# mdnunez/bayesflow_nddms

Hardware: AMD Instinct MI355X
Metric: simulated DDM trials/sec at n_trials=300 dt=0.001 (basic_ddm_dc, max_steps=4000) (higher is better)
Workload: dtype f32

## Files before the change

### bayesflow_nddms_amd/_lib.py

```python
import ctypes
import os

from .build import SO_PATH

NDDM_OK, NDDM_ERR_NULL, NDDM_ERR_SHAPE, NDDM_ERR_PARAM, NDDM_ERR_HIP, NDDM_ERR_NO_DEVICE = range(6)
GAUSS_EXACT, GAUSS_FAST, BRIDGE, GAUSS_PACKED, STATE_F64 = 0, 1, 2, 4, 8
QUANTILE_CONDITIONAL = 1
HMC_SIGMA_FIXED = 1
ABI_VERSION = 4

_lib = None


class NddmLibraryError(ImportError):
    pass


def _declare(L):
    c = ctypes
    fp, vp = c.c_void_p, c.c_void_p
    L.nddm_abi_version.restype = c.c_int
    L.nddm_last_error.restype = c.c_char_p
    L.nddm_device_count.argtypes = [c.POINTER(c.c_int)]
    L.nddm_set_device.argtypes = [c.c_int]
    L.nddm_summary_k.restype = c.c_int
    L.nddm_model_nparams.argtypes = [c.c_int]
    L.nddm_set_tuning.argtypes = [c.c_int] * 6
    L.nddm_set_debug_trace.argtypes = [c.c_void_p, c.c_int, c.c_int]
    L.nddm_set_ordering.argtypes = [c.c_int]
    L.nddm_debug_set_slot_limit.argtypes = [c.c_int]
    L.nddm_debug_last_launch.argtypes = [c.POINTER(c.c_int32)]
    common = [c.c_int64, c.c_int32, c.c_float, c.c_int32, c.c_uint64, c.c_uint64, c.c_uint32]
    for name in ("nddm_basic_ddm_dc_simulate", "nddm_single_trial_simulate", "nddm_single_trial_alt_simulate"):
        getattr(L, name).argtypes = [fp] + common + [fp, fp, vp]
    L.nddm_alpha_not_scaled_simulate.argtypes = [fp] + common + [c.c_float, c.c_int32, fp, fp, fp, vp]
    L.nddm_explicit_boundary_simulate.argtypes = [fp, fp] + common + [fp, fp, vp]
    L.nddm_simulratcliff.argtypes = [fp, c.c_int64, c.c_int32, c.c_uint64, c.c_uint64, c.c_uint32, c.c_float, c.c_int32, fp, fp, fp, vp]
    L.nddm_wiener_log_likelihood.argtypes = [c.c_int32, fp, c.c_int64, c.c_int64, fp, c.c_int32, c.c_uint32, fp, fp, vp]
    L.nddm_wiener_cdf.argtypes = [c.c_int32, fp, c.c_int64, c.c_int64, fp, c.c_int32, c.c_uint32, fp, fp, vp]
    L.nddm_wiener_log_likelihood_grad.argtypes = [c.c_int32, fp, c.c_int64, c.c_int64, fp, c.c_int32, c.c_uint32, fp, fp, vp]
    L.nddm_wiener_marginal_log_likelihood.argtypes = [c.c_int32, fp, c.c_int64, c.c_int64, fp, c.c_int32, c.c_float, c.c_uint32, fp, fp, vp]
    L.nddm_wiener_marginal_log_likelihood_grad.argtypes = [c.c_int32, fp, c.c_int64, c.c_int64, fp, c.c_int32, c.c_float, c.c_uint32, fp, fp, vp]
    L.nddm_wiener_hmc.argtypes = [c.c_int32, fp, c.c_int64, c.c_int32, c.c_int64, c.c_int64, fp, fp, c.c_int32, c.c_int32, c.c_int32, c.c_int32,
                                  c.c_uint32, c.c_uint64, c.c_uint64, c.c_uint64, c.c_uint32, fp, fp, fp, fp, fp, vp]
    L.nddm_wiener_hmc_joint.argtypes = [c.c_int32, fp, c.c_int64, c.c_int32, c.c_int64, c.c_int64, fp, fp, fp, fp, fp, c.c_int32, c.c_int32, c.c_int32,
                                        c.c_int32, c.c_uint32, c.c_uint64, c.c_uint64, c.c_uint64, c.c_uint32, fp, fp, fp, fp, fp, fp, fp, vp]
    L.nddm_wiener_quantile.argtypes = [c.c_int32, fp, c.c_int64, c.c_int64, fp, c.c_int32, c.c_uint32, fp, vp]
    L.nddm_simulate.argtypes = [c.c_int32, fp, fp] + common + [c.c_float, c.c_int32, fp, fp, fp, vp]
    L.nddm_simulate_indirect.argtypes = [c.c_int32, fp, fp] + common[:-1] + [fp, c.c_uint32, c.c_float, c.c_int32, fp, fp, fp, vp]
    L.nddm_simulate_codes.argtypes = [c.c_int32, fp] + common[:-1] + [fp, c.c_uint32, fp, fp, fp, vp]
    L.nddm_decode_codes.argtypes = [c.c_int32, fp, fp, c.c_int64, c.c_int32, c.c_float, fp, vp]
    L.nddm_draw_prior.argtypes = [c.c_int32, c.c_int64, c.c_uint64, c.c_uint64, c.c_float, fp, vp]
    L.nddm_draw_prior_indirect.argtypes = [c.c_int32, c.c_int64, c.c_uint64, c.c_uint64, fp, c.c_float, fp, vp]
    L.nddm_graph_arena_create.argtypes = [c.POINTER(c.c_uint64)]
    L.nddm_graph_arena_bind.argtypes = [c.c_uint64, c.POINTER(c.c_uint64)]
    L.nddm_graph_arena_info.argtypes = [c.c_uint64, c.POINTER(c.c_uint64), c.POINTER(c.c_int32)]
    L.nddm_graph_arena_release.argtypes = [c.c_uint64]
    L.nddm_source_hash.restype = c.c_char_p
    L.nddm_build_info.restype = c.c_char_p
    L.nddm_debug_normals.argtypes = [fp, c.c_int64, c.c_uint32, c.c_uint32, c.c_uint32, fp, vp]
    for name in EXPORTS:
        if name not in ("nddm_last_error", "nddm_source_hash", "nddm_build_info"):
            getattr(L, name).restype = c.c_int


EXPORTS = [
    "nddm_abi_version", "nddm_last_error", "nddm_device_count", "nddm_set_device", "nddm_summary_k",
    "nddm_model_nparams", "nddm_basic_ddm_dc_simulate", "nddm_single_trial_simulate",
    "nddm_single_trial_alt_simulate", "nddm_alpha_not_scaled_simulate", "nddm_explicit_boundary_simulate",
    "nddm_simulate", "nddm_draw_prior", "nddm_debug_normals", "nddm_set_tuning", "nddm_set_debug_trace", "nddm_set_ordering",
    "nddm_release_graph_memory", "nddm_debug_set_slot_limit", "nddm_debug_last_launch",
    "nddm_simulate_indirect", "nddm_draw_prior_indirect", "nddm_source_hash", "nddm_simulate_codes", "nddm_decode_codes",
    "nddm_graph_arena_create", "nddm_graph_arena_bind", "nddm_graph_arena_info", "nddm_graph_arena_release", "nddm_build_info",
    "nddm_simulratcliff", "nddm_wiener_log_likelihood", "nddm_wiener_cdf", "nddm_wiener_quantile",
    "nddm_wiener_log_likelihood_grad", "nddm_wiener_marginal_log_likelihood", "nddm_wiener_marginal_log_likelihood_grad",
    "nddm_wiener_hmc", "nddm_wiener_hmc_joint",
]


def lib():
    global _lib
    if _lib is None:
        from .build import build_hip, embedded_hash, is_stale, source_hash
        override = bool(os.environ.get("NDDM_HIP_LIB"))
        if is_stale():
            try:
                build_hip()
            except Exception as e:
                why = "is missing" if not os.path.exists(SO_PATH) else \
                    f"was built from other sources (library {embedded_hash()}, tree {source_hash()})"
                raise NddmLibraryError(
                    f"{SO_PATH} {why} and could not be rebuilt ({e!r}): build it with "
                    "`python -c 'import __graft_entry__ as g; g.build()'` (hipcc --offload-arch=gfx950).  "
                    "There is no CPU fallback.") from e
        if not os.path.exists(SO_PATH):
            raise NddmLibraryError(f"{SO_PATH} does not exist (NDDM_HIP_LIB points to a missing file?).  There is no CPU fallback.")
        import torch
        try:
            L = ctypes.CDLL(SO_PATH)
        except OSError as e:
            raise NddmLibraryError(f"cannot load {SO_PATH}: {e}") from e
        missing = [name for name in EXPORTS if not hasattr(L, name)]
        if missing:
            raise NddmLibraryError(f"{SO_PATH} does not export {missing}: it is older than this binding -- rebuild it "
                                   "(`python -c 'import __graft_entry__ as g; g.build()'`)")
        _declare(L)
        if L.nddm_abi_version() != ABI_VERSION:
            raise NddmLibraryError(f"ABI mismatch: library {L.nddm_abi_version()} != binding {ABI_VERSION} "
                                   "(the random stream differs between ABI versions): rebuild the library")
        if not override and L.nddm_source_hash().decode() != source_hash():
            raise NddmLibraryError(f"{SO_PATH} reports source hash {L.nddm_source_hash().decode()} but the tree hashes to "
                                   f"{source_hash()}: rebuild the library")
        _lib = L
    return _lib


def check(rc):
    if rc == NDDM_OK:
        return
    msg = lib().nddm_last_error().decode() or f"nddm status {rc}"
    if rc in (NDDM_ERR_NULL, NDDM_ERR_SHAPE, NDDM_ERR_PARAM):
        raise ValueError(msg)
    raise RuntimeError(msg)
```

### bayesflow_nddms_amd/build.py

```python
import hashlib
import os
import re
import shutil
import subprocess

_HERE = os.path.dirname(os.path.abspath(__file__))
SO_PATH = os.environ.get("NDDM_HIP_LIB") or os.path.join(_HERE, "libnddm_hip.so")
SOURCES = [os.path.join(_HERE, "csrc", "nddm_kernels.hip")]
HEADERS = [os.path.join(_HERE, "csrc", "nddm_rng.h"), os.path.join(_HERE, "csrc", "nddm_sim.h"),
           os.path.join(_HERE, "csrc", "nddm_prepass.h"), os.path.join(_HERE, "csrc", "nddm_ratcliff.h"),
           os.path.join(_HERE, "csrc", "nddm_wiener.h"), os.path.join(_HERE, "csrc", "nddm_wiener_cdf.h"),
           os.path.join(_HERE, "csrc", "nddm_wiener_quantile.h"), os.path.join(_HERE, "csrc", "nddm_wiener_grad.h"),
           os.path.join(_HERE, "csrc", "nddm_wiener_marginal.h"), os.path.join(_HERE, "csrc", "nddm_wiener_marginal_grad.h"),
           os.path.join(_HERE, "csrc", "nddm_wiener_hmc.h"),
           os.path.join(_HERE, "csrc", "nddm_wiener_hmc_joint.h"),
           os.path.join(os.path.dirname(_HERE), "include", "nddm.h")]
HIPCC_FLAGS = ["-O3", "-ffp-contract=off", "--offload-arch=gfx950", "-fPIC", "-shared", "-std=c++17"]


def _hipcc():
    exe = shutil.which("hipcc") or "/opt/rocm/bin/hipcc"
    if not os.path.exists(exe):
        raise RuntimeError("hipcc not found: the HIP extension cannot be built")
    return exe


def source_hash():
    h = hashlib.sha256()
    for p in SOURCES + HEADERS:
        h.update(os.path.basename(p).encode() + b"\0")
        with open(p, "rb") as f:
            h.update(f.read())
        h.update(b"\0")
    h.update(" ".join(HIPCC_FLAGS).encode())
    return h.hexdigest()


def embedded_hash(path=None):
    path = path or SO_PATH
    try:
        with open(path, "rb") as f:
            m = re.search(rb"NDDM_SRC_HASH=([0-9a-f]{64})", f.read())
# ... 89 lines not shown
```

### bayesflow_nddms_amd/csrc/nddm_kernels.hip

```cpp
#include <hip/hip_runtime.h>
#include <math.h>
#include <stdint.h>
#include <stdio.h>
#include <stdlib.h>
#include <string.h>

#include <mutex>
#include <thread>

#include "../../include/nddm.h"
#include "nddm_prepass.h"
#include "nddm_ratcliff.h"
#include "nddm_rng.h"
#include "nddm_sim.h"
#include "nddm_wiener.h"
#include "nddm_wiener_cdf.h"
#include "nddm_wiener_grad.h"
#include "nddm_wiener_hmc.h"
#include "nddm_wiener_hmc_joint.h"
#include "nddm_wiener_marginal.h"
#include "nddm_wiener_marginal_grad.h"
#include "nddm_wiener_quantile.h"

namespace nddm {

static thread_local char g_err[512] = "";

static int fail(int code, const char *fmt, const char *detail = "")
{
    snprintf(g_err, sizeof g_err, fmt, detail);
    return code;
}

static int round_up_pow2(int v) { int p = 1; while (p < v) p <<= 1; return p; }

static int check_stream(hipStream_t st)
{
    int sdev = -1, cur = -1;
    const hipError_t e = hipStreamGetDevice(st, &sdev);
    if (e != hipSuccess) {
        (void)hipGetLastError();
        return fail(NDDM_ERR_HIP, "`stream` is not a live stream of this process's HIP runtime (destroyed, or created by another copy "
                                  "of the runtime): %s", hipGetErrorString(e));
    }
    if (hipGetDevice(&cur) == hipSuccess && st != nullptr && st != hipStreamPerThread && sdev != cur)
        return fail(NDDM_ERR_PARAM, "`stream` belongs to another device than the current one (nddm_set_device / hipSetDevice)%s");
    return NDDM_OK;
}

struct Tuning { int sets_per_chunk, ring, refill_thresh, variant, grid_waves, tile_trials, no_order; };
struct LastLaunch { int grid_waves, vkeys, ring, tile_trials, tiles_per_set, sets_per_chunk, refill_thresh, lds_bytes; };
static thread_local LastLaunch g_last = {0, 0, 0, 0, 0, 0, 0, 0};
static std::mutex g_mu;
static Tuning g_tuning = {0, 0, 0, 0, 0, 0, 0};
static unsigned long long *g_dbg = nullptr;
static int g_dbg_waves = 0, g_dbg_chunks = 0;

constexpr int MAX_DEVICES = 64;
struct DeviceInfo { int cus = 0; double clock_hz = 0.0; };
static DeviceInfo g_dev[MAX_DEVICES];

static bool device_info(int dev, DeviceInfo *out)
{
    std::lock_guard<std::mutex> lock(g_mu);
    if (g_dev[dev].cus == 0) {
        hipDeviceProp_t prop;
        if (hipGetDeviceProperties(&prop, dev) != hipSuccess) return false;
        g_dev[dev].cus = prop.multiProcessorCount > 0 ? prop.multiProcessorCount : 1;
        g_dev[dev].clock_hz = prop.clockRate > 0 ? (double)prop.clockRate * 1e3 : 2.4e9;
    }
    *out = g_dev[dev];
    return true;
}

constexpr size_t SLOT_QUEUE_BYTES = 256, SLOT_SCRATCH = 1u << 20;
constexpr int MAX_SLOTS = 256;
struct LaunchSlot {
    char *base = nullptr;
    hipEvent_t done = nullptr;
    hipStream_t stream = nullptr;
    bool busy = false;
    bool fresh = true;
};
static LaunchSlot *g_slots[MAX_DEVICES][MAX_SLOTS];
static int g_nslots[MAX_DEVICES];
static int g_slot_limit = MAX_SLOTS;

static hipError_t malloc_relaxed(void **p, size_t bytes)
{
// ... 221 lines not shown
    }
    if (B < 0 || n_trials <= 0 || max_steps < 0) return fail(NDDM_ERR_SHAPE, "B < 0, n_trials <= 0 or max_steps < 0%s");
    if (max_steps >= (1 << 30)) return fail(NDDM_ERR_SHAPE, "max_steps must be < 2^30%s");
    if (set_offset >= (1ull << 60) || set_offset + (uint64_t)B > (1ull << 60))
        return fail(NDDM_ERR_SHAPE, "set_offset + B must be <= 2^60 (the random stream is keyed by 60 bits of the set index)%s");
    if (!(dt > 0.0f) || !isfinite(dt)) return fail(NDDM_ERR_PARAM, "dt must be finite and > 0%s");
    if (flags > 15u) return fail(NDDM_ERR_PARAM, "unknown flags%s");
    const bool bridge = (flags & NDDM_BRIDGE) != 0;
    const bool packed = (flags & NDDM_GAUSS_PACKED) != 0;
    const bool f64 = (flags & NDDM_STATE_F64) != 0;
    if (f64 && ((model != NDDM_BASIC_DDM_DC && model != NDDM_SINGLE_TRIAL) || bridge || packed || out_codes))
        return fail(NDDM_ERR_PARAM, "NDDM_STATE_F64 exists for NDDM_BASIC_DDM_DC and NDDM_SINGLE_TRIAL, without NDDM_BRIDGE, NDDM_GAUSS_PACKED "
                                    "or the 2-byte wire format%s");
    if (packed && (bridge || max_steps >= 16384))
        return fail(NDDM_ERR_PARAM, "NDDM_GAUSS_PACKED needs max_steps < 2^14 and cannot be combined with NDDM_BRIDGE%s");
    if (bridge && model != NDDM_ALPHA_NOT_SCALED)
        return fail(NDDM_ERR_PARAM, "NDDM_BRIDGE is only available for NDDM_ALPHA_NOT_SCALED%s");
    if (bridge && max_steps >= (1 << 22)) return fail(NDDM_ERR_SHAPE, "max_steps must be < 2^22 with NDDM_BRIDGE%s");
    if (B == 0) return NDDM_OK;
    if (!params) return fail(NDDM_ERR_NULL, "params is NULL%s");
    if (model == NDDM_EXPLICIT_BOUNDARY && !bounds) return fail(NDDM_ERR_NULL, "bounds is NULL%s");
    if (!out_trials && !out_summary && !out_ext && !out_codes) return fail(NDDM_ERR_NULL, "no output buffer given%s");
    if (out_codes && ((model != NDDM_BASIC_DDM_DC && model != NDDM_ALPHA_NOT_SCALED) || bridge || packed || max_steps >= 16384))
        return fail(NDDM_ERR_PARAM, "the 2-byte wire format exists for NDDM_BASIC_DDM_DC and NDDM_ALPHA_NOT_SCALED without NDDM_BRIDGE "
                                    "or NDDM_GAUSS_PACKED, max_steps < 2^14%s");
    if (B * (((long long)n_trials + 511) / 512) >= (1ll << 31))
        return fail(NDDM_ERR_SHAPE, "B * ceil(n_trials / 512) must be < 2^31 per launch%s");

    if (const int rc = check_stream(reinterpret_cast<hipStream_t>(stream))) return rc;

    Tuning tun;
    unsigned long long *dbg;
    int dbg_waves, dbg_chunks;
    { std::lock_guard<std::mutex> lock(g_mu); tun = g_tuning; dbg = g_dbg; dbg_waves = g_dbg_waves; dbg_chunks = g_dbg_chunks; }
    int dev = 0;
    {
        const hipError_t e = hipGetDevice(&dev);
        if (e != hipSuccess || dev < 0 || dev >= MAX_DEVICES) return fail(NDDM_ERR_HIP, "hipGetDevice: %s", hipGetErrorString(e));
    }
    DeviceInfo di;
    if (!device_info(dev, &di)) return fail(NDDM_ERR_HIP, "hipGetDeviceProperties failed%s");
    const int simds = 4 * di.cus;
    static const int sizing_per_simd = [] { const char *e = getenv("NDDM_SIZING_WAVES_PER_SIMD"); const int v = e ? atoi(e) : 0; return v >= 1 && v <= 8 ? v : 7; }();
    const long long waves_sizing = (long long)sizing_per_simd * simds;
    const long long waves_min_chunks = (long long)(sizing_per_simd - 1) * simds;

    SimArgs A;
    memset(&A, 0, sizeof A);
    A.params = params; A.bounds = bounds; A.out_trials = out_trials; A.out_summary = out_summary; A.out_ext = out_ext;
    A.out_codes = out_codes;
    A.B = B; A.n_trials = n_trials; A.max_k = max_steps; A.dt = dt; A.sqrt_dt = sqrtf(dt);
    A.tscale = bridge ? dt * 0.00390625f : dt;
    A.k0 = (uint32_t)seed; A.k1 = (uint32_t)(seed >> 32);
    A.ext_sigma = ext_sigma; A.ext_mode = ext_mode;
    A.dbg = dbg; A.dbg_waves = dbg_waves; A.dbg_chunks = dbg_chunks;
    A.dt64 = (double)dt; A.sqrt_dt64 = sqrt((double)dt);

    const bool res16 = (flags & NDDM_BRIDGE) == 0 && max_steps < 16384;
    const size_t per_trial = res16 ? 2 : 4;
    const long long total_trials = B * (long long)n_trials;
    double est_steps = 0.25 / (double)dt;
    if (est_steps > (double)max_steps) est_steps = (double)max_steps;
    if (est_steps < 1.0) est_steps = 1.0;
    const double est_blocks = (double)total_trials * est_steps / 256.0;
    long long plan_waves = 8ll * simds;
    if (tun.grid_waves > 0) plan_waves = tun.grid_waves;
    else {
        const double cap_blocks = max_steps > 4 ? (double)max_steps * 0.25 : 1.0;
        double want = est_blocks / 300.0;
        const double crit = 3.0 * (double)simds * pow(est_blocks / cap_blocks / (2.8 * (double)simds), 0.4);
        if (crit < want) want = crit;
        if (want < (double)plan_waves) plan_waves = want < (double)simds ? simds : (long long)want;
    }
    const long long waves_for_tiles = plan_waves < waves_sizing ? plan_waves : waves_sizing;
    int tile_cap = 64;
    while (tile_cap < 512 && (long long)tile_cap * waves_for_tiles * 8 < total_trials) tile_cap <<= 1;
    int tiles = tun.tile_trials > 0 ? (n_trials + tun.tile_trials - 1) / tun.tile_trials
                                    : (n_trials <= tile_cap ? 1 : (n_trials + tile_cap - 1) / tile_cap);
    int tile_n = (n_trials + tiles - 1) / tiles;
    tiles = (n_trials + tile_n - 1) / tile_n;
    if (!tun.ring && !tun.tile_trials)
        while (tile_n > 96 && (size_t)lds_header_bytes(model) + 4u * (size_t)slot_stride_bytes(tile_n, (int)per_trial) > 5120u) {
            tiles++;
            tile_n = (n_trials + tiles - 1) / tiles;
            tiles = (n_trials + tile_n - 1) / tile_n;
        }
    const long long vB = B * (long long)tiles;
    if (vB >= (1ll << 31)) return fail(NDDM_ERR_SHAPE, "B * ceil(n_trials / 512) must be < 2^31 per launch%s");
// ... 254 lines not shown
int nddm_set_device(int device)
{
    const hipError_t e = hipSetDevice(device);
    if (e != hipSuccess) return nddm::fail(NDDM_ERR_HIP, "hipSetDevice: %s", hipGetErrorString(e));
    return NDDM_OK;
}

int nddm_set_tuning(int sets_per_chunk, int ring, int refill_thresh, int variant, int grid_waves, int tile_trials)
{
    if (ring < 0 || ring == 1) return nddm::fail(NDDM_ERR_PARAM, "ring must be 0 (automatic) or >= 2%s");
    std::lock_guard<std::mutex> lock(nddm::g_mu);
    const int no_order = nddm::g_tuning.no_order;
    nddm::g_tuning = {sets_per_chunk, ring, refill_thresh, variant < 0 ? 0 : variant, grid_waves, tile_trials, no_order};
    return NDDM_OK;
}

int nddm_set_ordering(int enabled)
{
    std::lock_guard<std::mutex> lock(nddm::g_mu);
    nddm::g_tuning.no_order = enabled ? 0 : 1;
    return NDDM_OK;
}

int nddm_set_debug_trace(void *dev_u64, int wave_capacity, int chunk_capacity)
{
    if (dev_u64 && (wave_capacity < 0 || chunk_capacity < 0)) return nddm::fail(NDDM_ERR_PARAM, "negative trace capacity%s");
    std::lock_guard<std::mutex> lock(nddm::g_mu);
    nddm::g_dbg = static_cast<unsigned long long *>(dev_u64);
    nddm::g_dbg_waves = dev_u64 ? wave_capacity : 0;
    nddm::g_dbg_chunks = dev_u64 ? chunk_capacity : 0;
    return NDDM_OK;
}

int nddm_debug_last_launch(int32_t *out8)
{
    if (!out8) return nddm::fail(NDDM_ERR_NULL, "out8 is NULL%s");
    const nddm::LastLaunch &l = nddm::g_last;
    out8[0] = l.grid_waves; out8[1] = l.vkeys; out8[2] = l.ring; out8[3] = l.tile_trials; out8[4] = l.tiles_per_set;
    out8[5] = l.sets_per_chunk; out8[6] = l.refill_thresh; out8[7] = l.lds_bytes;
    return NDDM_OK;
}

int nddm_debug_set_slot_limit(int n)
{
    std::lock_guard<std::mutex> lock(nddm::g_mu);
    nddm::g_slot_limit = n < 1 ? 1 : (n > nddm::MAX_SLOTS ? nddm::MAX_SLOTS : n);
    return NDDM_OK;
}

int nddm_release_graph_memory(void)
{
    nddm::g_err[0] = 0;
    int dev = 0;
    const hipError_t e = hipGetDevice(&dev);
    if (e != hipSuccess || dev < 0 || dev >= nddm::MAX_DEVICES) return nddm::fail(NDDM_ERR_HIP, "hipGetDevice: %s", hipGetErrorString(e));
    nddm::GraphAlloc *mine = nullptr;
    {
        std::lock_guard<std::mutex> lock(nddm::g_mu);
        nddm::GraphAlloc **pp = &nddm::g_ownerless.list;
        while (*pp) {
            nddm::GraphAlloc *a = *pp;
            if (a->dev == dev) { *pp = a->next; a->next = mine; mine = a; }
            else pp = &a->next;
        }
    }
    nddm::free_list(mine);
// ... 438 lines not shown
```

### bayesflow_nddms_amd/csrc/nddm_sim.h

```cpp
#pragma once
#include <hip/hip_runtime.h>
#include <math.h>
#include <stdint.h>

#include "../../include/nddm.h"
#include "nddm_rng.h"

namespace nddm {

constexpr int WAVE = 64;
constexpr int MAX_REJECT = 64;

typedef __attribute__((address_space(3))) uint16_t lds_u16;
typedef __attribute__((address_space(3))) uint32_t lds_u32;
typedef uint32_t u32v4 __attribute__((ext_vector_type(4)));
typedef uint32_t u32v2 __attribute__((ext_vector_type(2)));
typedef __attribute__((address_space(3))) u32v4 lds_u32v4;
typedef __attribute__((address_space(3))) u32v2 lds_u32v2;

template <int MODEL> struct ModelTraits;
template <> struct ModelTraits<NDDM_BASIC_DDM_DC>      { static constexpr int P = 5; static constexpr bool HAS_Z = false; static constexpr int TAU = 3; };
template <> struct ModelTraits<NDDM_SINGLE_TRIAL>      { static constexpr int P = 8; static constexpr bool HAS_Z = true;  static constexpr int TAU = 3; };
template <> struct ModelTraits<NDDM_SINGLE_TRIAL_ALT>  { static constexpr int P = 8; static constexpr bool HAS_Z = true;  static constexpr int TAU = 3; };
template <> struct ModelTraits<NDDM_ALPHA_NOT_SCALED>  { static constexpr int P = 6; static constexpr bool HAS_Z = false; static constexpr int TAU = 3; };
template <> struct ModelTraits<NDDM_EXPLICIT_BOUNDARY> { static constexpr int P = 4; static constexpr bool HAS_Z = true;  static constexpr int TAU = 2; };

struct SimArgs {
    const float *params;
    const float *bounds;
    float *out_trials;
    float *out_summary;
    float *out_ext;
    uint16_t *out_codes;
    long long B;
    int n_trials;
    int n_total;
    int tiles_per_set;
    unsigned long long *partials;
    const uint32_t *recs;
    int max_k;
    float dt;
    float sqrt_dt;
    float tscale;
    uint32_t k0, k1;
    int sets_per_chunk;
    int n_chunks;
    unsigned int *chunk_counter;
    int ring;
    int open_ahead;
    float ext_sigma;
    int ext_mode;
    unsigned long long *dbg;
    int dbg_waves, dbg_chunks;
    int res16;
    int refill_thresh;
    uint32_t ring_magic;
    double dt64, sqrt_dt64;
};

typedef const __attribute__((address_space(4))) SimArgs *ArgsPtr;
__device__ __forceinline__ ArgsPtr fresh_args(ArgsPtr p)
{
    asm volatile("" : "+s"(p));
    return p;
}

template <bool FAST>
struct AuxStream {
    uint32_t trial, set_lo, c3, blk, kbase;
    u32x4 x;
    __device__ __forceinline__ AuxStream(uint32_t kbase_, uint32_t set_lo_, uint32_t set_hi28, uint32_t trial_)
        : trial(trial_), set_lo(set_lo_), c3(set_hi28 | 0x10000000u), blk(0xffffffffu), kbase(kbase_) {}
    __device__ __forceinline__ void block(uint32_t b)
    {
        if (b != blk) { x = philox4x32_10_lds(set_lo, trial, c3, b, kbase); blk = b; }
    }
    __device__ __forceinline__ void first_pair(float &z0, float &z1)
    {
        block(0u);
        float r, cs, sn;
        polar_pair<FAST>(x.x, x.y, r, cs, sn);
        r *= noise_unit<FAST>(1.0f);
        z0 = r * cs; z1 = r * sn;
    }
    __device__ __forceinline__ float normal(uint32_t a)
    {
        block(a >> 2);
        const bool second = (a & 2u) != 0u;
        float r, cs, sn;
        polar_pair<FAST>(second ? x.z : x.x, second ? x.w : x.y, r, cs, sn);
        r *= noise_unit<FAST>(1.0f);
        return r * ((a & 1u) ? sn : cs);
    }
};

__device__ __forceinline__ unsigned long long wave_sum(unsigned long long v)
{
#pragma unroll
    for (int off = 32; off > 0; off >>= 1) v += __shfl_xor(v, off, WAVE);
    return v;
}
__device__ __forceinline__ int wave_sum(int v)
{
#pragma unroll
    for (int off = 32; off > 0; off >>= 1) v += __shfl_xor(v, off, WAVE);
    return v;
}

__device__ __forceinline__ int fresh_lane(int lane)
{
    asm volatile("" : "+v"(lane));
    return lane;
}

__device__ __forceinline__ uint32_t lane_rank(unsigned long long mask)
{
    return __builtin_amdgcn_mbcnt_hi((uint32_t)(mask >> 32), __builtin_amdgcn_mbcnt_lo((uint32_t)mask, 0u));
}

__device__ __forceinline__ void finalize_summary(float *o, int n_up, int n_lo, int n_miss, unsigned long long sk,
                                                 unsigned long long sk2, unsigned long long sk_up,
                                                 unsigned long long sk2_up, long long sz, long long szz, int n_total,
                                                 float tscale, float tau)
{
    const double dtd = (double)tscale, taud = (double)tau;
    const double n_resp = (double)(n_up + n_lo);
    o[0] = (float)n_up; o[1] = (float)n_lo; o[2] = (float)n_miss;
    if (n_resp > 0) {
        const double mk = (double)sk / n_resp;
        const double vk = (double)sk2 / n_resp - mk * mk;
        o[3] = (float)(taud + dtd * mk);
        o[4] = (float)(dtd * dtd * vk);
    } else { o[3] = __builtin_nanf(""); o[4] = __builtin_nanf(""); }
    if (n_up > 0) {
        const double nu = (double)n_up;
        const double mk = (double)sk_up / nu;
        const double vk = (double)sk2_up / nu - mk * mk;
        o[5] = (float)(taud + dtd * mk);
        o[6] = (float)(dtd * dtd * vk);
    } else { o[5] = __builtin_nanf(""); o[6] = __builtin_nanf(""); }
    const double Nd = (double)n_total;
    const double mz = ((double)sz / 4294967296.0) / Nd;
    const double vz = ((double)szz / 16777216.0) / Nd - mz * mz;
    o[7] = (float)mz;
    o[8] = (float)vz;
// ... 266 lines not shown
        const int s0 = ring_slot(t, R->ring, R->ring_magic);
        const int o0 = s0 * stride, o01 = (s0 + 1 == R->ring ? 0 : s0 + 1) * stride - o0;
        return (o0 & 0xffff) | (o01 << 16);
    };
    constexpr uint32_t SLOTS_OFF = lds_header_bytes(MODEL);
    constexpr uint32_t FIFO_OFF = LDS_HEADER_DWORDS * 4;
    [[maybe_unused]] int fifo_pos = 0, fifo_avail = 0;

    float w = 0.0f, h = 0.0f, mu_dt = 0.0f;
    [[maybe_unused]] double xe = 0.0, ab = 0.0, cdt = 0.0, sdc = 0.0;
    int k = 0;
    [[maybe_unused]] float ta = 0.0f, tb = 0.0f;
    [[maybe_unused]] uint32_t jraw = 0;
    uint32_t res_addr = 0;
    [[maybe_unused]] int tile = 0;
    bool invalid = false;
    unsigned long long has_m = 0ull, act_m = 0ull;
    constexpr int MAX_BLOCKS = 16;
    [[maybe_unused]] int cap_k = -1;
    PathCtr pc = {0u, 0u, 0u, 0u, 0u};
    [[maybe_unused]] PathKeys pkeys;
    if constexpr (VKEYS) pkeys.init(A.k0, A.k1);

    int tile_open = 0;
    int flushed = 0;
    int next_tile = 0, next_trial = 0;
    int to_retire = N;
    int chunk_set = 0, chunk_left = 0;
    int slot_pack = pack_slots(0);
    int dirty = 1;
    unsigned long long dbg_cnt = 0;
    unsigned long long *dbg_stamp = reinterpret_cast<unsigned long long *>(lds_raw + 20);
    if (lane == 0) {
        dbg_stamp[3] = 0;
        lds_raw[31] = blockIdx.x;
        if (Ak->dbg) { dbg_stamp[0] = __builtin_amdgcn_s_memtime(); dbg_stamp[1] = __builtin_amdgcn_s_memrealtime(); }
    }

    uint32_t pre = 0u;

    auto open_tiles = [&]() {
        const ArgsPtr R = fresh_args(Ak);
        while (tile_open < flushed + R->ring && tile_open <= next_tile + R->open_ahead) {
            const bool have_pre = chunk_left > 0;
            if (chunk_left <= 0) {
                if (chunk_left < 0) break;
                unsigned int c = 0;
                if (fresh_lane(lane) == 0) c = atomicAdd(R->chunk_counter, 1u);
                c = __builtin_amdgcn_readfirstlane(c);
                if (c >= (unsigned int)R->n_chunks) {
                    chunk_left = -1;
                    if (fresh_lane(lane) == 0 && R->dbg) dbg_stamp[3] = __builtin_amdgcn_s_memrealtime();
                    break;
                }
                if (fresh_lane(lane) == 0 && R->dbg && c < (unsigned int)R->dbg_chunks)
                    R->dbg[8ll * R->dbg_waves + c] = __builtin_amdgcn_s_memrealtime();
                chunk_set = (int)c * R->sets_per_chunk;
                const long long left = R->B - (long long)chunk_set;
                chunk_left = (int)(left < R->sets_per_chunk ? left : R->sets_per_chunk);
            }
            const int slot = ring_slot(tile_open, R->ring, R->ring_magic);
            const int TPS = R->tiles_per_set;
            const int prow = TPS == 1 ? chunk_set : chunk_set / TPS;
            const int qt = chunk_set - prow * TPS;
            uint32_t rec = pre;
            if (!have_pre) rec = fresh_lane(lane) < REC ? R->recs[(long long)prow * REC + lane] : 0u;
// ... 165 lines not shown
                } else if constexpr (MODEL == NDDM_SINGLE_TRIAL_ALT) {
                    const float sig_c = latent;
                    const float inv_t = 1.0f / noise_unit<FAST>(H->sqrt_dt * sig_c);
                    const float hv = 0.5f * a1;
                    mu_dt = (a0 * H->dt) * inv_t;
                    h = hv * inv_t;
                    w = (a1 * a2 - hv) * inv_t;
                } else if constexpr (MODEL == NDDM_ALPHA_NOT_SCALED) {
                    mu_dt = latent;
                    h = a2; w = a3;
                } else if constexpr (MODEL == NDDM_EXPLICIT_BOUNDARY) {
                    const float a = trial < (uint32_t)H->n_total ? H->bounds[(long long)d2.x * H->n_total + trial] : 1.0f;
                    invalid = !(a >= 0.0f);
                    const float hv = 0.5f * a;
                    mu_dt = a0;
                    h = invalid ? 0.0f : hv * a1;
                    w = (a * a2 - hv) * a1;
                }
                const uint4 kq = *reinterpret_cast<const uint4 *>(lds_raw + 28);
                pc.init(d1.x, d1.y, d1.z, d1.w, trial, kq.x, kq.y, kq.z);
                k = 0;
                if constexpr (BRIDGE) { ta = h - __builtin_fabsf(w); tb = ta; jraw = 0u; }
            }
            if constexpr (LATENT) { const int n_ok = (int)__popcll(ok_mask); fifo_pos += n_ok; fifo_avail -= n_ok; }
            if constexpr (BRIDGE) act_m = __builtin_amdgcn_ballot_w64(ta > 0.0f) & __builtin_amdgcn_ballot_w64(k < A.max_k) & has_m;
            else if constexpr (F64) act_m = __builtin_amdgcn_ballot_w64(xe > 0.0) & __builtin_amdgcn_ballot_w64(xe < ab) & __builtin_amdgcn_ballot_w64(k < A.max_k) & has_m;
            else if constexpr (CAP4 && !PACKED) {
                const int max_k = fresh_args(Ak)->max_k;
                act_m = max_k > 0 ? __builtin_amdgcn_ballot_w64(in_range(w, h)) & has_m : 0ull;
                const int near_from = A.refill_thresh < WAVE ? max_k - 4 * MAX_BLOCKS : (int)0x80000000;
                cap_k = (__builtin_amdgcn_ballot_w64(k >= near_from) & has_m) ? max_k : -1;
            }
            else act_m = __builtin_amdgcn_ballot_w64(in_range(w, h)) & __builtin_amdgcn_ballot_w64(k < A.max_k) & has_m;
        }
        const int it_limit = A.refill_thresh < WAVE ? MAX_BLOCKS - 1 : 0x7fffffff;
        const int occupied = (int)__popcll(has_m);
        const int leave_at = occupied < A.refill_thresh ? occupied : A.refill_thresh;
        int it = 0;
        for (;; ++it) {
            if constexpr (BRIDGE) {
                const uint32_t blk = (uint32_t)k;
                const u32x4 u4 = philox4x32_10_path(blk | 0x80000000u, pc, kbase);
                unsigned long long &live = act_m;
#pragma unroll
                for (int half = 0; half < 2; ++half) {
                    const u32x4 rb = philox4x32_10_path(blk + 4u * (uint32_t)half, pc, kbase);
                    float r0, r1, c0, c1, c2, c3;
                    polar_pair<FAST, true>(rb.x, rb.y, r0, c0, c1);
                    polar_pair<FAST, true>(rb.z, rb.w, r1, c2, c3);
                    const uint32_t ua = half ? u4.z : u4.x, ub = half ? u4.w : u4.y;
                    if constexpr (FAST && CAP4) {
                        float m, uf;
#define NDDM_BSTEP(R, T, D0, D1, CVT, KLIT) "v_fmac_f32 %[w], %[" R "], %[" T "]\n\tv_add_f32 %[w], %[mu], %[w]\n\tv_sub_f32 %[" D1 "], %[h], |%[w]|\n\t" \
    "v_mul_f32 %[m], %[" D0 "], %[" D1 "]\n\tv_fmaak_f32 %[m], -4.0, %[m], " KLIT "\n\tv_exp_f32 %[m], %[m]\n\t" CVT                        \
    "v_cmpx_ge_f32_e64 vcc, %[uf], %[m]\n\tv_add_u32 %[k], 1, %[k]\n\t"
#define NDDM_U32(W) "v_cvt_f32_u32 %[uf], %[" W "]\n\t"
#define NDDM_U16(W) "v_and_b32 %[uf], 0xffff, %[" W "]\n\tv_cvt_f32_u32 %[uf], %[uf]\n\t"
                        asm volatile("s_mov_b64 exec, %[lm]\n\t"
                                     "v_mov_b32 %[jr], %[ua]\n\t"
                                     NDDM_BSTEP("r0", "c0", "ta", "tb", NDDM_U32("ua"), "0x42000001")
                                     NDDM_BSTEP("r0", "c1", "tb", "ta", NDDM_U16("ua"), "0x41800000")
                                     "v_mov_b32 %[jr], %[ub]\n\t"
                                     NDDM_BSTEP("r1", "c2", "ta", "tb", NDDM_U32("ub"), "0x42000001")
                                     NDDM_BSTEP("r1", "c3", "tb", "ta", NDDM_U16("ub"), "0x41800000")
                                     "s_nop 1\n\ts_mov_b64 %[lm], exec\n\ts_mov_b64 exec, -1"
                                     : [w] "+v"(w), [k] "+v"(k), [ta] "+v"(ta), [tb] "+v"(tb), [jr] "+v"(jraw), [lm] "+s"(live), [m] "=&v"(m),
// ... 100 lines not shown
                             "2:"
                             : [w] "+v"(w), [k] "+v"(k), [am] "+s"(act_m)
                             : [ck] "s"(cap_k), [mu] "v"(mu_dt), [h] "v"(h), [r0] "v"(rr[0]), [r1] "v"(rr[2]),
                               [t0] "v"(tt[0]), [t1] "v"(tt[1]), [t2] "v"(tt[2]), [t3] "v"(tt[3])
                             : "vcc", "scc");
#undef NDDM_STEP
#undef NDDM_K2
                if ((int)__popcll(has_m & ~act_m) >= leave_at) break;
                if (it >= it_limit) break;
                continue;
            }
#pragma unroll
            for (int j = 0; j < NS; ++j) {
                if (active) {
                    asm volatile("" ::: "memory");
                    w = __builtin_fmaf(rr[j], tt[j], w) + mu_dt;
                    k++;
                    if (j < NS - 1) {
                        if constexpr (CAP4) active = in_range(w, h);
                        else active = in_range(w, h) && (k < A.max_k);
                    }
                }
            }
            act_m = __builtin_amdgcn_ballot_w64(in_range(w, h)) & __builtin_amdgcn_ballot_w64(k < A.max_k) & has_m;
            if ((int)__popcll(has_m & ~act_m) >= leave_at) break;
            if (it >= it_limit) break;
        }
        dbg_cnt += (1ull << 32) | (unsigned long long)(uint32_t)(it + 1);
    }
    if (lane == 0) {
        unsigned int *const q = fresh_args(Ak)->chunk_counter;
        const unsigned int left = atomicAdd(q + 1, 1u);
        if (left == gridDim.x - 1u) { atomicExch(q, 0u); atomicExch(q + 1, 0u); }
    }
    unsigned long long *const dbg = fresh_args(Ak)->dbg;
    if (dbg && lane == 0) {
        const unsigned long long t_end = __builtin_amdgcn_s_memrealtime(), c_end = __builtin_amdgcn_s_memtime();
        const uint32_t wg = lds_raw[31];
        if (wg < (uint32_t)fresh_args(Ak)->dbg_waves) {
            unsigned long long *const r = dbg + 8ull * wg;
            r[0] = dbg_cnt & 0xffffffffull; r[1] = dbg_cnt >> 32;
            r[2] = c_end - dbg_stamp[0]; r[3] = t_end - dbg_stamp[1];
            r[4] = dbg_stamp[1]; r[5] = dbg_stamp[3]; r[6] = t_end; r[7] = 1ull;
        }
    }
}

}
```

### include/nddm.h

```cpp
#ifndef NDDM_H
#define NDDM_H

#include <stdint.h>

#ifdef __cplusplus
extern "C" {
#endif

#define NDDM_ABI_VERSION 4
#define NDDM_SUMMARY_K 10

enum nddm_summary_col {
    NDDM_S_N_UPPER = 0,
    NDDM_S_N_LOWER = 1,
    NDDM_S_N_MISSING = 2,
    NDDM_S_MEAN_RT = 3,
    NDDM_S_VAR_RT = 4,
    NDDM_S_MEAN_RT_UPPER = 5,
    NDDM_S_VAR_RT_UPPER = 6,
    NDDM_S_MEAN_Z = 7,
    NDDM_S_VAR_Z = 8,
    NDDM_S_CHOICE_MEAN = 9
};

// ... 8 lines not shown
enum nddm_status {
    NDDM_OK = 0,
    NDDM_ERR_NULL = 1,
    NDDM_ERR_SHAPE = 2,
    NDDM_ERR_PARAM = 3,
    NDDM_ERR_HIP = 4,
    NDDM_ERR_NO_DEVICE = 5
};

enum nddm_flags {
    NDDM_GAUSS_EXACT = 0,
    NDDM_GAUSS_FAST = 1,
    NDDM_GAUSS_PACKED = 4,
    NDDM_STATE_F64 = 8,
    NDDM_BRIDGE = 2
};

int nddm_abi_version(void);
const char *nddm_last_error(void);
int nddm_device_count(int *count);
int nddm_set_device(int device);
int nddm_summary_k(void);
int nddm_model_nparams(int model);
int nddm_graph_arena_create(uint64_t *arena);
int nddm_graph_arena_bind(uint64_t arena, uint64_t *previous );
int nddm_graph_arena_info(uint64_t arena, uint64_t *bytes , int32_t *n_allocations );
int nddm_graph_arena_release(uint64_t arena);
int nddm_release_graph_memory(void);
int nddm_debug_set_slot_limit(int n);
int nddm_debug_last_launch(int32_t *out8);
int nddm_set_tuning(int sets_per_chunk, int ring, int refill_thresh, int variant, int grid_waves, int tile_trials);
int nddm_set_ordering(int enabled);
int nddm_set_debug_trace(void *dev_u64, int wave_capacity, int chunk_capacity);


int nddm_basic_ddm_dc_simulate(const float *params, int64_t B, int32_t n_trials, float dt, int32_t max_steps,
                               uint64_t seed, uint64_t set_offset, uint32_t flags, float *out_trials,
                               float *out_summary, void *stream);

int nddm_single_trial_simulate(const float *params, int64_t B, int32_t n_trials, float dt, int32_t max_steps,
                               uint64_t seed, uint64_t set_offset, uint32_t flags, float *out_trials,
                               float *out_summary, void *stream);

int nddm_single_trial_alt_simulate(const float *params, int64_t B, int32_t n_trials, float dt, int32_t max_steps,
                                   uint64_t seed, uint64_t set_offset, uint32_t flags, float *out_trials,
                                   float *out_summary, void *stream);

int nddm_alpha_not_scaled_simulate(const float *params, int64_t B, int32_t n_trials, float dt, int32_t max_steps,
                                   uint64_t seed, uint64_t set_offset, uint32_t flags, float ext_sigma,
                                   int32_t ext_mode, float *out_trials, float *out_summary, float *out_extdata,
                                   void *stream);

int nddm_simulratcliff(const float *params, int64_t B, int32_t n_trials, uint64_t seed, uint64_t set_offset, uint32_t flags,
                       float ext_sigma, int32_t ext_mode, float *out_trials, float *out_summary, float *out_extdata, void *stream);

int nddm_wiener_log_likelihood(int32_t model, const float *params, int64_t R, int64_t draws_per_dataset, const float *data,
                               int32_t n_trials, uint32_t flags, float *out_trial_logp ,
                               double *out_loglik , void *stream);

int nddm_wiener_log_likelihood_grad(int32_t model, const float *params, int64_t R, int64_t draws_per_dataset, const float *data,
                                    int32_t n_trials, uint32_t flags , double *out_loglik ,
                                    double *out_grad , void *stream);

int nddm_wiener_hmc(int32_t model, const float *data , int64_t D, int32_t n_trials, int64_t C,
                    int64_t chains_per_dataset, double *state , const double *inv_mass , int32_t n_iter,
                    int32_t n_adapt, int32_t n_leapfrog, int32_t thin, uint32_t free_mask, uint64_t seed, uint64_t chain_offset,
// ... 66 lines not shown
```

Measured before the change: 9.576 billion.

## Fan out straggler trials across the wave during the tail phase

When a wave has no more chunks to fetch and only a few lanes (default up to two) still hold unfinished trials, the whole wave now advances one straggler at a time. All 64 lanes generate Philox normals for consecutive future steps of that trial's counter stream, and a serial scan over the broadcast values finds the boundary crossing. This targets the long-tail cost where nearly idle waves step single trials one step per iteration. It adds readlane-heavy scan code, a tunable mode and lane threshold, and a pass counter. It relies on the counter-based RNG to keep the same random stream, but the exact crossing step depends on the scan matching the original per-step update.

Result: no change. 9.575 billion (median of 2 runs) (-0.0%).

```diff
diff --git a/bayesflow_nddms_amd/_lib.py b/bayesflow_nddms_amd/_lib.py
--- a/bayesflow_nddms_amd/_lib.py
+++ b/bayesflow_nddms_amd/_lib.py
@@ -27,6 +27,8 @@
     L.nddm_model_nparams.argtypes = [c.c_int]
     L.nddm_set_tuning.argtypes = [c.c_int] * 6
     L.nddm_set_debug_trace.argtypes = [c.c_void_p, c.c_int, c.c_int]
+    if hasattr(L, "nddm_set_tail_fanout"):
+        L.nddm_set_tail_fanout.argtypes = [c.c_int, c.c_int, c.c_void_p]
     L.nddm_set_ordering.argtypes = [c.c_int]
     L.nddm_debug_set_slot_limit.argtypes = [c.c_int]
     L.nddm_debug_last_launch.argtypes = [c.POINTER(c.c_int32)]
@@ -60,15 +62,18 @@
     L.nddm_build_info.restype = c.c_char_p
     L.nddm_debug_normals.argtypes = [fp, c.c_int64, c.c_uint32, c.c_uint32, c.c_uint32, fp, vp]
     for name in EXPORTS:
-        if name not in ("nddm_last_error", "nddm_source_hash", "nddm_build_info"):
+        if name not in ("nddm_last_error", "nddm_source_hash", "nddm_build_info") and hasattr(L, name):
             getattr(L, name).restype = c.c_int
 
+
+ADDITIVE = ("nddm_set_tail_fanout",)
 
 EXPORTS = [
     "nddm_abi_version", "nddm_last_error", "nddm_device_count", "nddm_set_device", "nddm_summary_k",
     "nddm_model_nparams", "nddm_basic_ddm_dc_simulate", "nddm_single_trial_simulate",
     "nddm_single_trial_alt_simulate", "nddm_alpha_not_scaled_simulate", "nddm_explicit_boundary_simulate",
     "nddm_simulate", "nddm_draw_prior", "nddm_debug_normals", "nddm_set_tuning", "nddm_set_debug_trace", "nddm_set_ordering",
+    "nddm_set_tail_fanout",
     "nddm_release_graph_memory", "nddm_debug_set_slot_limit", "nddm_debug_last_launch",
     "nddm_simulate_indirect", "nddm_draw_prior_indirect", "nddm_source_hash", "nddm_simulate_codes", "nddm_decode_codes",
     "nddm_graph_arena_create", "nddm_graph_arena_bind", "nddm_graph_arena_info", "nddm_graph_arena_release", "nddm_build_info",
@@ -100,7 +105,7 @@
             L = ctypes.CDLL(SO_PATH)
         except OSError as e:
             raise NddmLibraryError(f"cannot load {SO_PATH}: {e}") from e
-        missing = [name for name in EXPORTS if not hasattr(L, name)]
+        missing = [name for name in EXPORTS if not hasattr(L, name) and not (override and name in ADDITIVE)]
         if missing:
             raise NddmLibraryError(f"{SO_PATH} does not export {missing}: it is older than this binding -- rebuild it "
                                    "(`python -c 'import __graft_entry__ as g; g.build()'`)")
diff --git a/bayesflow_nddms_amd/build.py b/bayesflow_nddms_amd/build.py
--- a/bayesflow_nddms_amd/build.py
+++ b/bayesflow_nddms_amd/build.py
@@ -8,6 +8,7 @@
 SO_PATH = os.environ.get("NDDM_HIP_LIB") or os.path.join(_HERE, "libnddm_hip.so")
 SOURCES = [os.path.join(_HERE, "csrc", "nddm_kernels.hip")]
 HEADERS = [os.path.join(_HERE, "csrc", "nddm_rng.h"), os.path.join(_HERE, "csrc", "nddm_sim.h"),
+           os.path.join(_HERE, "csrc", "nddm_tail_scan.h"),
            os.path.join(_HERE, "csrc", "nddm_prepass.h"), os.path.join(_HERE, "csrc", "nddm_ratcliff.h"),
            os.path.join(_HERE, "csrc", "nddm_wiener.h"), os.path.join(_HERE, "csrc", "nddm_wiener_cdf.h"),
            os.path.join(_HERE, "csrc", "nddm_wiener_quantile.h"), os.path.join(_HERE, "csrc", "nddm_wiener_grad.h"),
diff --git a/bayesflow_nddms_amd/csrc/nddm_kernels.hip b/bayesflow_nddms_amd/csrc/nddm_kernels.hip
--- a/bayesflow_nddms_amd/csrc/nddm_kernels.hip
+++ b/bayesflow_nddms_amd/csrc/nddm_kernels.hip
@@ -55,6 +55,9 @@
 static Tuning g_tuning = {0, 0, 0, 0, 0, 0, 0};
 static unsigned long long *g_dbg = nullptr;
 static int g_dbg_waves = 0, g_dbg_chunks = 0;
+constexpr int TAIL_FANOUT_LANES = 2;
+static int g_fan_mode = 0, g_fan_lanes = 0;
+static unsigned long long *g_fan_count = nullptr;
 
 constexpr int MAX_DEVICES = 64;
 struct DeviceInfo { int cus = 0; double clock_hz = 0.0; };
@@ -342,7 +345,13 @@
     Tuning tun;
     unsigned long long *dbg;
     int dbg_waves, dbg_chunks;
-    { std::lock_guard<std::mutex> lock(g_mu); tun = g_tuning; dbg = g_dbg; dbg_waves = g_dbg_waves; dbg_chunks = g_dbg_chunks; }
+    int fan_mode, fan_lanes;
+    unsigned long long *fan_count;
+    {
+        std::lock_guard<std::mutex> lock(g_mu);
+        tun = g_tuning; dbg = g_dbg; dbg_waves = g_dbg_waves; dbg_chunks = g_dbg_chunks;
+        fan_mode = g_fan_mode; fan_lanes = g_fan_lanes; fan_count = g_fan_count;
+    }
     int dev = 0;
     {
         const hipError_t e = hipGetDevice(&dev);
@@ -364,6 +373,8 @@
     A.k0 = (uint32_t)seed; A.k1 = (uint32_t)(seed >> 32);
     A.ext_sigma = ext_sigma; A.ext_mode = ext_mode;
     A.dbg = dbg; A.dbg_waves = dbg_waves; A.dbg_chunks = dbg_chunks;
+    A.fan_max = fan_mode == 1 ? 0 : (fan_mode == 2 ? WAVE : (fan_lanes > 0 ? fan_lanes : TAIL_FANOUT_LANES));
+    A.fan_count = fan_count;
     A.dt64 = (double)dt; A.sqrt_dt64 = sqrt((double)dt);
 
     const bool res16 = (flags & NDDM_BRIDGE) == 0 && max_steps < 16384;
@@ -684,6 +695,16 @@
     return NDDM_OK;
 }
 
+int nddm_set_tail_fanout(int mode, int max_lanes, void *dev_u64_passes)
+{
+    if (mode < 0 || mode > 2 || max_lanes < 0 || max_lanes > nddm::WAVE)
+        return nddm::fail(NDDM_ERR_PARAM, "mode must be 0 (rule), 1 (never) or 2 (whenever eligible), max_lanes 0..64%s");
+    std::lock_guard<std::mutex> lock(nddm::g_mu);
+    nddm::g_fan_mode = mode; nddm::g_fan_lanes = max_lanes;
+    nddm::g_fan_count = static_cast<unsigned long long *>(dev_u64_passes);
+    return NDDM_OK;
+}
+
 int nddm_debug_last_launch(int32_t *out8)
 {
     if (!out8) return nddm::fail(NDDM_ERR_NULL, "out8 is NULL%s");
diff --git a/bayesflow_nddms_amd/csrc/nddm_sim.h b/bayesflow_nddms_amd/csrc/nddm_sim.h
--- a/bayesflow_nddms_amd/csrc/nddm_sim.h
+++ b/bayesflow_nddms_amd/csrc/nddm_sim.h
@@ -5,6 +5,7 @@
 
 #include "../../include/nddm.h"
 #include "nddm_rng.h"
+#include "nddm_tail_scan.h"
 
 namespace nddm {
 
@@ -56,6 +57,8 @@
     int refill_thresh;
     uint32_t ring_magic;
     double dt64, sqrt_dt64;
+    int fan_max;
+    unsigned long long *fan_count;
 };
 
 typedef const __attribute__((address_space(4))) SimArgs *ArgsPtr;
@@ -111,6 +114,23 @@
 {
     asm volatile("" : "+v"(lane));
     return lane;
+}
+
+__device__ __forceinline__ uint32_t lane_bcast(uint32_t v, int s)
+{
+    const uint32_t x = (uint32_t)__builtin_amdgcn_readlane((int)v, s);
+    uint32_t r;
+    asm("v_mov_b32 %0, %1" : "=v"(r) : "s"(x));
+    return r;
+}
+__device__ __forceinline__ float lane_read(float v, int s)
+{
+    return __int_as_float(__builtin_amdgcn_readlane(__float_as_int(v), s));
+}
+
+__host__ __device__ constexpr bool tail_fanout_model(int model)
+{
+    return model >= 0;
 }
 
 __device__ __forceinline__ uint32_t lane_rank(unsigned long long mask)
@@ -443,6 +463,7 @@
     unsigned long long dbg_cnt = 0;
     unsigned long long *dbg_stamp = reinterpret_cast<unsigned long long *>(lds_raw + 20);
     if (lane == 0) {
+        dbg_stamp[2] = 0;
         dbg_stamp[3] = 0;
         lds_raw[31] = blockIdx.x;
         if (Ak->dbg) { dbg_stamp[0] = __builtin_amdgcn_s_memtime(); dbg_stamp[1] = __builtin_amdgcn_s_memrealtime(); }
@@ -674,6 +695,49 @@
                 cap_k = (__builtin_amdgcn_ballot_w64(k >= near_from) & has_m) ? max_k : -1;
             }
             else act_m = __builtin_amdgcn_ballot_w64(in_range(w, h)) & __builtin_amdgcn_ballot_w64(k < A.max_k) & has_m;
+        }
+        if constexpr (CAP4 && !PACKED && !BRIDGE && !F64 && tail_fanout_model(MODEL)) {
+            if (chunk_left <= 0 && next_tile >= tile_open && act_m != 0ull) {
+                const ArgsPtr R = fresh_args(Ak);
+                if (chunk_left == 0 && (int)__popcll(act_m) <= R->fan_max && tile_open < flushed + R->ring) { dirty = 1; continue; }
+                if (chunk_left < 0 && (int)__popcll(act_m) <= R->fan_max) {
+                    const int max_k = R->max_k;
+                    const int pass_limit = (max_k >> 8) + 1;
+                    uint32_t passes = 0;
+                    for (int n = 0; n < WAVE && act_m != 0ull; ++n) {
+                        const int s = (int)__builtin_ctzll(act_m);
+                        PathCtr pcs;
+                        pcs.cA = lane_bcast(pc.cA, s); pcs.cB = lane_bcast(pc.cB, s); pcs.cC = lane_bcast(pc.cC, s);
+                        pcs.cD = lane_bcast(pc.cD, s); pcs.cE = lane_bcast(pc.cE, s);
+                        const float mus = lane_read(mu_dt, s), hs = lane_read(h, s);
+                        float ws = lane_read(w, s);
+                        int ks = __builtin_amdgcn_readlane(k, s);
+                        for (int p = 0; p < pass_limit; ++p) {
+                            const uint32_t draw = (uint32_t)ks + 4u * (uint32_t)lane;
+                            u32x4 rb;
+                            if constexpr (VKEYS) rb = philox4x32_10_path(draw, pcs, pkeys);
+                            else rb = philox4x32_10_path(draw, pcs, kbase);
+                            float g_r0, g_t0, g_t1, g_r1, g_t2, g_t3;
+                            polar_pair<FAST, true>(rb.x, rb.y, g_r0, g_t0, g_t1);
+                            polar_pair<FAST, true>(rb.z, rb.w, g_r1, g_t2, g_t3);
+                            const TailScan sc = tail_scan(
+                                [&](int b, float &r0, float &t0, float &t1, float &r1, float &t2, float &t3) {
+                                    r0 = lane_read(g_r0, b); t0 = lane_read(g_t0, b); t1 = lane_read(g_t1, b);
+                                    r1 = lane_read(g_r1, b); t2 = lane_read(g_t2, b); t3 = lane_read(g_t3, b);
+                                },
+                                ws, ks, mus, hs, max_k);
+                            ws = sc.w; ks = sc.k;
+                            passes++;
+                            if (sc.ended) break;
+                        }
+                        if (fresh_lane(lane) == s) { w = ws; k = ks; }
+                        act_m &= ~(1ull << s);
+                    }
+                    dbg_cnt += (1ull << 32) | (unsigned long long)passes;
+                    if (fresh_lane(lane) == 0) dbg_stamp[2] += passes;
+                    continue;
+                }
+            }
         }
         const int it_limit = A.refill_thresh < WAVE ? MAX_BLOCKS - 1 : 0x7fffffff;
         const int occupied = (int)__popcll(has_m);
@@ -840,6 +904,8 @@
         unsigned int *const q = fresh_args(Ak)->chunk_counter;
         const unsigned int left = atomicAdd(q + 1, 1u);
         if (left == gridDim.x - 1u) { atomicExch(q, 0u); atomicExch(q + 1, 0u); }
+        unsigned long long *const fc = fresh_args(Ak)->fan_count;
+        if (fc && dbg_stamp[2]) atomicAdd(fc, dbg_stamp[2]);
     }
     unsigned long long *const dbg = fresh_args(Ak)->dbg;
     if (dbg && lane == 0) {
diff --git a/bayesflow_nddms_amd/csrc/nddm_tail_scan.h b/bayesflow_nddms_amd/csrc/nddm_tail_scan.h
--- /dev/null
+++ b/bayesflow_nddms_amd/csrc/nddm_tail_scan.h
@@ -0,0 +1,55 @@
+#pragma once
+
+#if defined(__HIPCC__) || defined(__CUDACC__)
+#define NDDM_TAIL_HD __host__ __device__ __forceinline__
+#else
+#define NDDM_TAIL_HD inline
+#endif
+
+#if defined(__HIP_DEVICE_COMPILE__)
+#define NDDM_TAIL_MASK(c) __builtin_amdgcn_ballot_w64(c)
+#else
+#define NDDM_TAIL_MASK(c) ((unsigned long long)(c))
+#endif
+
+namespace nddm {
+
+constexpr int TAIL_BLOCKS = 64;
+
+struct TailScan {
+    float w;
+    int k;
+    bool ended;
+    int blocks;
+};
+
+template <class Fetch>
+NDDM_TAIL_HD TailScan tail_scan(Fetch fetch, float w, int k, float mu, float h, int max_k)
+{
+    TailScan s = {w, k, false, 0};
+    for (int b = 0; b < TAIL_BLOCKS; ++b) {
+        float r0, t0, t1, r1, t2, t3;
+        fetch(b, r0, t0, t1, r1, t2, t3);
+        s.blocks = b + 1;
+        const float w1 = __builtin_fmaf(r0, t0, s.w) + mu;
+        const float w2 = __builtin_fmaf(r0, t1, w1) + mu;
+        const float w3 = __builtin_fmaf(r1, t2, w2) + mu;
+        const float w4 = __builtin_fmaf(r1, t3, w3) + mu;
+        const unsigned long long i1 = NDDM_TAIL_MASK(__builtin_fabsf(w1) < h), i2 = NDDM_TAIL_MASK(__builtin_fabsf(w2) < h);
+        const unsigned long long i3 = NDDM_TAIL_MASK(__builtin_fabsf(w3) < h), i4 = NDDM_TAIL_MASK(__builtin_fabsf(w4) < h);
+        if ((i1 & i2 & i3 & i4) != 0ull) {
+            s.w = w4; s.k += 4;
+            if (s.k >= max_k) { s.ended = true; break; }
+            continue;
+        }
+        s.ended = true;
+        if (!i1) { s.w = w1; s.k += 1; }
+        else if (!i2) { s.w = w2; s.k += 2; }
+        else if (!i3) { s.w = w3; s.k += 3; }
+        else { s.w = w4; s.k += 4; }
+        break;
+    }
+    return s;
+}
+
+}
diff --git a/include/nddm.h b/include/nddm.h
--- a/include/nddm.h
+++ b/include/nddm.h
@@ -64,6 +64,7 @@
 int nddm_set_tuning(int sets_per_chunk, int ring, int refill_thresh, int variant, int grid_waves, int tile_trials);
 int nddm_set_ordering(int enabled);
 int nddm_set_debug_trace(void *dev_u64, int wave_capacity, int chunk_capacity);
+int nddm_set_tail_fanout(int mode, int max_lanes, void *dev_u64_passes);
 
 
 int nddm_basic_ddm_dc_simulate(const float *params, int64_t B, int32_t n_trials, float dt, int32_t max_steps,
```
